# wpats/scanner

Hardware: AMD Instinct MI355X
Metric: Msamples/s (complex samples through convert->window->FFT->dB->threshold) (higher is better)
Workload: dtype f32

## Files before the change

scanner_amd/build.py:

```python
import os
import shutil
import subprocess
import sys

HERE = os.path.dirname(os.path.abspath(__file__))
CSRC = os.path.join(HERE, "csrc")
LIB = os.path.join(HERE, "libscanner_hip.so")
SOURCES = ["scn_kernels.hip", "scn_mixed.hip", "scn_generic.hip", "scn_big.hip", "scn_hits.hip", "scn_floor.hip", "scn_floor_local.hip", "scn_baseline.hip", "scn_welch.hip", "scn_average.hip", "scn_gather.hip", "scn_host.hip", "scn_plan.hip", "scn_submit.hip",
           "scn_collect.hip", "scn_welch_plan.hip"]
HEADERS = ["scn_kernels.h", "scn_mask.h", "scn_wire.h", "scn_dispatch.h", "scn_host.h", "scn_plan.h", "scn_resource.h", "scn_device.h", "scn_detect.h", "scn_mixed_dft.h", "scn_mixed_plans.h", "scn_sizes.h", "scn_gather_protocol.h", os.path.join("..", "..", "include", "scanner_hip.h")]
ARCH = "gfx950"
EXTRA_FLAGS = ["-fvisibility=hidden", "-fvisibility-inlines-hidden", "-DSCN_BUILDING_LIBRARY"]
PUBLIC_HEADER = os.path.join(HERE, "..", "include", "scanner_hip.h")
MAP_FILE = os.path.join(HERE, "libscanner_hip.map")
LINK_FLAGS = ["-Wl,--version-script=" + MAP_FILE]


def declared_symbols():
    import re

    with open(PUBLIC_HEADER) as fh:
        text = re.sub(r"/\*.*?\*/", "", fh.read(), flags=re.S)
    return sorted(set(re.findall(r"\bSCN_API\b[^;{]*?\b(scn_\w+)\s*\(", text)))


def write_map():
    with open(MAP_FILE, "w") as fh:
        fh.write("{\n  global:\n" + "".join(f"    {n};\n" for n in declared_symbols()) + "  local:\n    *;\n};\n")
SPLIT = {"scn_kernels.hip": ("SCN_TU", 8), "scn_mixed.hip": ("SCN_MIXED_TU", 8), "scn_average.hip": ("SCN_AVG_TU", 4)}


def hipcc():
    exe = shutil.which("hipcc") or "/opt/rocm/bin/hipcc"
    if not os.path.exists(exe):
        raise RuntimeError("hipcc not found; the HIP path cannot be built")
    return exe


def source_hash():
    import hashlib

    h = hashlib.sha256()
    for f in sorted(SOURCES + HEADERS):
        with open(os.path.join(CSRC, f), "rb") as fh:
            h.update(f.encode() + b"\0" + fh.read())
    with open(os.path.abspath(__file__), "rb") as fh:
        h.update(b"build.py\0" + fh.read())
    return h.hexdigest()[:16]


HASH_FILE = LIB + ".hash"


def _stale():
    if not os.path.exists(LIB) or not os.path.exists(HASH_FILE):
        return True
    with open(HASH_FILE) as fh:
        return fh.read().strip() != source_hash()


def build(force=False, verbose=False, defines=(), out=None):
    target = out or LIB
    if not out and not force and not _stale():
        return LIB
    import fcntl

    with open(LIB + ".lock", "w") as lock:
        fcntl.flock(lock, fcntl.LOCK_EX)
        if not out and not force and not _stale():
            return LIB
        return _build_locked(target, verbose, defines, out)


def _build_locked(target, verbose, defines, out):
    built_from = source_hash()
    write_map()
    objs, cmds = [], []
    tag = "" if not out else "." + os.path.basename(out).replace(".so", "")
    units = [(src, None) for src in SOURCES if src not in SPLIT] + [(src, tu) for src, (_, count) in SPLIT.items() for tu in range(count)]
    for src, tu in sorted(units, key=lambda u: u[1] is None):
        suffix = tag + ("" if tu is None else f".tu{tu}") + ".o"
        obj = os.path.join(os.path.dirname(out) if out else CSRC, src.replace(".hip", suffix))
        cmd = [hipcc(), f"--offload-arch={ARCH}", "-O3", "-std=c++17", "-fPIC", "-Wall", "-Wno-unused-function", "-Wno-unused-const-variable",
               "-fno-slp-vectorize", *EXTRA_FLAGS, *[f"-D{d}" for d in defines], *([] if tu is None else [f"-D{SPLIT[src][0]}={tu}"]),
               "-c", os.path.join(CSRC, src), "-o", obj]
        if verbose:
            print(" ".join(cmd), file=sys.stderr)
        cmds.append(cmd)
        objs.append(obj)
    from concurrent.futures import ThreadPoolExecutor

    with ThreadPoolExecutor(max_workers=min(len(cmds), os.cpu_count() or 1)) as pool:
        list(pool.map(subprocess.check_call, cmds))
    cmd = [hipcc(), f"--offload-arch={ARCH}", "-shared", "-fPIC", *LINK_FLAGS, "-o", target] + objs + ["-ldl"]
    if verbose:
        print(" ".join(cmd), file=sys.stderr)
    subprocess.check_call(cmd)
    if not out:
        with open(HASH_FILE, "w") as fh:
            fh.write(built_from + "\n")
    return target


HOST = os.path.join(HERE, "host")
HOST_LIB = os.path.join(HERE, "libscanner_host.so")
HOST_DEMO = os.path.join(HOST, "scan_synth")
ABI_BENCH = os.path.join(HOST, "abi_bench")
HOST_SOURCES = ["frequencyTable.cpp", "messageQueue.cpp", "captureWriter.cpp", "signalSource.cpp", "syntheticSource.cpp", "fileSource.cpp",
                "processInterface.cpp", "sampleBuffer.cpp", "process.cpp"]


def build_host(force=False, verbose=False):
    build(force=False)
    srcs = [os.path.join(HOST, f) for f in HOST_SOURCES]
    deps = srcs + [os.path.join(HOST, f) for f in os.listdir(HOST) if f.endswith(".h")] + [LIB]
    if force or not os.path.exists(HOST_LIB) or any(os.path.getmtime(d) > os.path.getmtime(HOST_LIB) for d in deps):
        cmd = ["g++", "-std=gnu++11", "-O2", "-g", "-fPIC", "-shared", "-Wall", "-pthread", "-o", HOST_LIB] + srcs + \
              ["-L" + HERE, "-lscanner_hip", "-Wl,-rpath,$ORIGIN"]
        if verbose:
            print(" ".join(cmd), file=sys.stderr)
        subprocess.check_call(cmd)
    demo_src = os.path.join(HOST, "scan_synth.cpp")
    if force or not os.path.exists(HOST_DEMO) or \
            max(os.path.getmtime(demo_src), os.path.getmtime(HOST_LIB)) > os.path.getmtime(HOST_DEMO):
        cmd = ["g++", "-std=gnu++11", "-O2", "-g", "-Wall", "-pthread", "-o", HOST_DEMO, demo_src, "-L" + HERE,
               "-lscanner_host", "-lscanner_hip", "-Wl,-rpath,$ORIGIN/.."]
        if verbose:
            print(" ".join(cmd), file=sys.stderr)
        subprocess.check_call(cmd)
    bench_src = os.path.join(HOST, "abi_bench.cpp")
    if force or not os.path.exists(ABI_BENCH) or os.path.getmtime(bench_src) > os.path.getmtime(ABI_BENCH) or \
            os.path.getmtime(os.path.join(HERE, "..", "include", "scanner_hip.h")) > os.path.getmtime(ABI_BENCH):
        rocm = os.environ.get("ROCM_PATH", "/opt/rocm")
        cmd = ["g++", "-std=gnu++11", "-O2", "-g", "-Wall", "-D__HIP_PLATFORM_AMD__", "-I" + os.path.join(rocm, "include"), "-o", ABI_BENCH,
               bench_src, "-L" + os.path.join(rocm, "lib"), "-lamdhip64", "-ldl", "-Wl,-rpath," + os.path.join(rocm, "lib")]
        if verbose:
            print(" ".join(cmd), file=sys.stderr)
        subprocess.check_call(cmd)
    return HOST_LIB, HOST_DEMO


if __name__ == "__main__":
    build_host(force="--force" in sys.argv, verbose=True)
    print(build(force="--force" in sys.argv, verbose=True))
```

scanner_amd/csrc/scn_kernels.hip:

```cpp
#include <hip/hip_runtime.h>
#include <hip/hip_ext.h>
#include <stdint.h>
#include <stdlib.h>

#include "scn_device.h"
#include "scn_dispatch.h"
#include "scn_kernels.h"

#ifndef SCN_TU
#define SCN_TU -1
#endif
#define SCN_IN_TU(x) (SCN_TU == -1 || SCN_TU == (x))
#define SCN_TU_COUNT 8


#define SCN_WORK_QUEUE_SETUP()                                                                         \
  const uint32_t wq_shard = blockIdx.x & 7u;                                                           \
  uint32_t *const wq_head = args.work_counter + 32u * wq_shard;        \
  const uint32_t wq_base = args.work_base[wq_shard];                                                   \
  const uint32_t wq_j0 = (gridDim.x - wq_shard + 7u) >> 3;                                             \
  uint32_t wq_zero;                                                                                    \
  asm("v_mov_b32 %0, 0" : "=v"(wq_zero));                                                              \
  auto wq_take = [&]() -> uint32_t { return atomicAdd(wq_head + wq_zero, 1u); };                       \
  auto wq_buffer = [&](uint32_t taken) -> uint32_t { return 8u * (wq_j0 + (taken - wq_base)) + wq_shard; }

template <int M, int KIND, bool DC, bool HITS, bool SPEC>
__global__ __launch_bounds__(16 * M, Geo<M>::WAVES_PER_SIMD) void scn_fft_kernel(ScnFftArgs args) {
  static_assert(HITS || SPEC, "a kernel that reports nothing");
  typedef Geo<M> G;
  constexpr int AUX_LD = SCN_AUX_LD;
  constexpr int AUX_ST = SCN_AUX_ST;
  constexpr bool DYN = scn_uses_queue(KIND, G::N);
  constexpr uint32_t N = G::N, T = G::T, P1 = G::P1, P2 = G::P2;
  typedef RawLoader<KIND> L;
  extern __shared__ __attribute__((aligned(16))) char smem_raw[];
  v2f *lds = reinterpret_cast<v2f *>(smem_raw);
  v2f *lds_tw2 = lds + G::EXCH;
  int *lds_cnt = reinterpret_cast<int *>(lds_tw2 + T);
  int *lds_hits = lds_cnt + 32;
  uint32_t *lds_next = reinterpret_cast<uint32_t *>(lds_hits + 2);

  const uint32_t t = threadIdx.x;
  const uint32_t p2 = t / M, c2 = t % M;
  const uint32_t lane = t & 63, wave = t >> 6;

  typename L::raw_t raw[16];
  if (blockIdx.x < args.n_buffers) {
    __amdgpu_buffer_rsrc_t r0 = make_rsrc(reinterpret_cast<const char *>(args.raw) + (size_t)blockIdx.x * L::kBytes * N, L::kBytes * N);
#pragma unroll
    for (int a = 0; a < 16; a++) raw[a] = L::template load<AUX_LD>(r0, N, t, T * a);
  }

  cf tw1[16];
#pragma unroll
  for (int p = 1; p < 16; p++) tw1[p] = from_v2f(args.tw1_table[(p - 1) * T + t]);
  float win[16];
#pragma unroll
  for (int a = 0; a < 16; a++) win[a] = args.window[T * a + t] * args.scale;
  lds_tw2[t] = args.twiddle[(16 * p2 * c2) & (N - 1)];
  SCN_WORK_QUEUE_SETUP();
  if (t == 0) {
    lds_hits[0] = lds_hits[1] = 0;
    lds_next[0] = DYN ? wq_buffer(wq_take()) : blockIdx.x + gridDim.x;
  }
  __syncthreads();

  v2f *w1 = lds + t;
  v2f *r1 = lds + p2 * P1 + c2;
  v2f *w2 = lds + c2 * P2 + p2;
  v2f *r3 = lds + t;
  const v2f *tw2 = lds_tw2 + c2;
  const uint32_t st_voff = t * 4u;

  auto joff_of = [](int o) -> uint32_t { return T * ((uint32_t)o / M) + 256u * ((uint32_t)o % M); };
  uint32_t keepmask = 0;
  if (HITS) {
#pragma unroll
    for (int o = 0; o < 16; o++) {
      const uint32_t j = t + joff_of(o);
      const uint32_t i = j ^ (N / 2);
      const bool keep = scn_bin_evaluated(j, i, N, args);
      keepmask |= keep ? (1u << o) : 0u;
    }
  }
  uint32_t par = 0;
  uint32_t prev = 0xffffffffu;

  uint32_t buf = blockIdx.x;
  uint32_t nxt = (uint32_t)__builtin_amdgcn_readfirstlane((int)lds_next[0]);
  while (buf < args.n_buffers) {
    const bool more = nxt < args.n_buffers;
    int dc_re = 0, dc_im = 0;
    if (DC) {
      int sr = 0, si = 0;
#pragma unroll
      for (int a = 0; a < 16; a++) {
        int re, im;
        L::ints(raw[a], re, im);
        sr += re;
        si += im;
      }
      sr = wave_sum(sr);
      si = wave_sum(si);
      if (lane == 0) {
        lds_cnt[wave] = sr;
        lds_cnt[16 + wave] = si;
      }
      __syncthreads();
      sr = si = 0;
#pragma unroll
      for (uint32_t w = 0; w < G::WAVES; w++) {
        sr += lds_cnt[w];
        si += lds_cnt[16 + w];
      }
      dc_re = (int)((uint32_t)sr / N);
      dc_im = (int)((uint32_t)si / N);
    }

    cf v[16];
#pragma unroll
    for (int a = 0; a < 16; a++) v[a] = L::conv(raw[a], dc_re, dc_im, 1.0f) * win[a];
    uint32_t taken = 0;
    if (DYN && t == 0 && more) taken = wq_take();
    const __amdgpu_buffer_rsrc_t rn =
        make_rsrc(reinterpret_cast<const char *>(args.raw) + (size_t)(more ? nxt : buf) * (L::kBytes * N), more ? L::kBytes * N : 0u);
    auto prefetch = [&](int a_lo, int a_hi) {
#pragma unroll
      for (int a = 0; a < 16; a++)
        if (a >= a_lo && a < a_hi) raw[a] = L::template load<AUX_LD>(rn, N, t, T * a);
    };
    prefetch(0, 6);

    fft16(v);
#pragma unroll
    for (int p = 0; p < 16; p++) {
      cf y = v[OUT16(p)];
      if (p) y = cmul(y, tw1[p]);
      w1[p * P1] = to_v2f(y);
    }
    __syncthreads();
    if (HITS) {
      if (t == 0 && prev != 0xffffffffu) {
        args.per_buffer_hits[prev] = (uint32_t)lds_hits[par ^ 1];
        if (args.host_hits) args.host_hits[prev] = (uint32_t)lds_hits[par ^ 1];
        lds_hits[par ^ 1] = 0;
      }
    }

#pragma unroll
    for (int b = 0; b < 16; b++) v[b] = from_v2f(r1[b * M]);
    prefetch(6, 11);
    fft16(v);
#pragma unroll
    for (int q = 1; q < 16; q++) v[OUT16(q)] = cmul(v[OUT16(q)], from_v2f(tw2[q * M]));
    __syncthreads();
    prefetch(11, 16);
#pragma unroll
    for (int q = 0; q < 16; q++) w2[q * 16] = to_v2f(v[OUT16(q)]);
    __syncthreads();

#pragma unroll
    for (int u = 0; u < 16 / M; u++)
#pragma unroll
      for (int c = 0; c < M; c++) v[u * M + c] = from_v2f(r3[c * P2 + T * u]);
    if constexpr (M == 16) fft16(v);
    if constexpr (M == 8) {
      fft8(v);
      fft8(v + 8);
    }
    if constexpr (M == 4) {
#pragma unroll
      for (int u = 0; u < 4; u++) radix4(v[4 * u], v[4 * u + 1], v[4 * u + 2], v[4 * u + 3]);
    }

    v16f pw;
    float gmax[4] = {0.0f, 0.0f, 0.0f, 0.0f};
    __amdgpu_buffer_rsrc_t rout = make_rsrc(args.power_db + (size_t)buf * N, (SPEC && args.power_db) ? 4u * N : 0u);
#pragma unroll
    for (int o = 0; o < 16; o++) {
      const float q = power_of(v[out_reg<M>(o)]);
      pw[o] = q;
      gmax[o >> 2] = fmaxf(gmax[o >> 2], q);
      if constexpr (SPEC) __builtin_amdgcn_raw_buffer_store_b32(__builtin_bit_cast(int, db_fast(q)), rout, st_voff, 4u * joff_of(o), AUX_ST);
    }
    const float pmax = fmaxf(fmaxf(gmax[0], gmax[1]), fmaxf(gmax[2], gmax[3]));
    if constexpr (SPEC) scn_store_exact_db<16>(pw, gmax, pmax, rout, st_voff, [&](int o) -> uint32_t { return 4u * joff_of(o); });
    if (t == 0) lds_next[0] = !more ? 0xffffffffu : DYN ? wq_buffer(taken) : nxt + gridDim.x;
    __syncthreads();
    const uint32_t after = (uint32_t)__builtin_amdgcn_readfirstlane((int)lds_next[0]);
    if (HITS) {
      if (__ballot(pmax > args.p_lo))
        scn_record_hits_lanes<16, false, true>(pw, gmax, keepmask, args, &lds_hits[par], buf, lane, [&](int o) -> uint32_t { return (t + joff_of(o)) ^ (N / 2); });
      prev = buf;
      par ^= 1;
    }
    buf = nxt;
    nxt = after;
  }
  if (HITS) {
    __syncthreads();
    if (t == 0 && prev != 0xffffffffu) {
      args.per_buffer_hits[prev] = (uint32_t)lds_hits[par ^ 1];
      if (args.host_hits) args.host_hits[prev] = (uint32_t)lds_hits[par ^ 1];
    }
  }
}

namespace {
template <int T, bool SPEC, bool HITS, typename POWER, typename JOFF, typename STORE>
__device__ __forceinline__ void scn_small_db_store_record(POWER power_at, JOFF joff_of, STORE store, const ScnFftArgs &args, uint32_t buf, bool valid,
                                                          uint32_t keepmask, uint32_t t, uint32_t n) {
  v16f pw, dbv;
  float gmax[4] = {0.0f, 0.0f, 0.0f, 0.0f};
#pragma unroll
  for (int o = 0; o < 16; o++) {
    const float q = power_at(o);
    pw[o] = q;
    gmax[o >> 2] = fmaxf(gmax[o >> 2], q);
    if constexpr (SPEC) {
      const float d = db_fast(q);
      dbv[o] = d;
      store(o, d, true);
    }
  }
  const float pmax = fmaxf(fmaxf(gmax[0], gmax[1]), fmaxf(gmax[2], gmax[3]));
  const bool any_cand = HITS && __ballot(valid && pmax > args.p_lo) != 0ull;
  if (SPEC || any_cand) {
    if constexpr (!SPEC) {
#pragma unroll
      for (int o = 0; o < 16; o++) dbv[o] = db_fast(pw[o]);
    }
    if (__ballot(pmax >= SCN_P_EXACT_FROM)) {
#pragma unroll
      for (int g = 0; g < 4; g++) {
        if (__ballot(gmax[g] >= SCN_P_EXACT_FROM)) {
#pragma unroll
          for (int o = 4 * g; o < 4 * g + 4; o++) {
            const float q = pw[o];
            if (__ballot(q >= SCN_P_EXACT_FROM)) {
              const float d = db_exact(q);
              dbv[o] = q >= SCN_P_EXACT_FROM ? d : dbv[o];
              if constexpr (SPEC) store(o, d, q >= SCN_P_EXACT_FROM);
            }
          }
        }
      }
    }
  }
  if constexpr (HITS) {
    uint32_t total = 0;
    if (any_cand) {
      uint32_t hm = 0;
#pragma unroll
      for (int o = 0; o < 16; o++) hm |= (dbv[o] > args.threshold) ? (1u << o) : 0u;
      hm &= valid ? keepmask : 0u;
      total = scn_record_hits_segment<T, 16>(dbv, hm, args, buf, t, [&](int o) -> uint32_t { return (t + joff_of(o)) ^ (n / 2); });
    }
    if (t == 0 && valid) {
      args.per_buffer_hits[buf] = total;
      if (args.host_hits) args.host_hits[buf] = total;
    }
  }
}

template <int M>
struct GeoSmall {
  static constexpr uint32_t N = 256u * M, T = 16u * M, SLOTS = 256u / T;
  static constexpr uint32_t P1 = T + M, P2 = 256u + 16u / M;
  static constexpr uint32_t EXCH = (16u * P1 > M * P2) ? 16u * P1 : M * P2;
  static constexpr uint32_t LDS_BYTES = SLOTS * EXCH * 8u + T * 8u + 16u;
  static constexpr uint32_t WG_PER_CU = 3;
};
}

template <int M, int KIND, bool DC, bool HITS, bool SPEC>
__global__ __launch_bounds__(256, 3) void scn_fft_small_kernel(ScnFftArgs args) {
  static_assert(M == 1 || M == 2, "256 or 512 points");
  static_assert(HITS || SPEC, "a kernel that reports nothing");
  typedef GeoSmall<M> G;
  constexpr int AUX_LD = SCN_AUX_LD;
  constexpr int AUX_ST = SCN_AUX_ST;
  constexpr uint32_t N = G::N, T = G::T, SLOTS = G::SLOTS, P1 = G::P1, P2 = G::P2;
  typedef RawLoader<KIND> L;
  extern __shared__ __attribute__((aligned(16))) char smem_raw[];
  const uint32_t tid = threadIdx.x, t = tid % T, slot = tid / T;
  v2f *lds = reinterpret_cast<v2f *>(smem_raw) + slot * G::EXCH;
  v2f *lds_tw2 = reinterpret_cast<v2f *>(smem_raw) + SLOTS * G::EXCH;
  const uint32_t p2 = t / M, c2 = t % M;
  const uint32_t buf_bytes = L::kBytes * N;

  auto in_rsrc = [&](uint32_t first) {
    const bool ok = first < args.n_buffers;
    const uint32_t nb = ok ? (args.n_buffers - first < SLOTS ? args.n_buffers - first : SLOTS) : 0u;
    return make_rsrc(reinterpret_cast<const char *>(args.raw) + (size_t)(ok ? first : 0u) * buf_bytes, nb * buf_bytes);
  };
  typename L::raw_t raw[16];
  auto load_group = [&](const __amdgpu_buffer_rsrc_t &r, int a_lo, int a_hi) {
#pragma unroll
    for (int a = 0; a < 16; a++)
      if (a >= a_lo && a < a_hi) raw[a] = L::template load<AUX_LD>(r, N, t + slot * (KIND == SCN_K_SHORT ? 2u * N : N), T * a);
  };
  uint32_t first = blockIdx.x * SLOTS;
  load_group(in_rsrc(first), 0, 16);

  cf tw1[16];
#pragma unroll
  for (int p = 1; p < 16; p++) tw1[p] = from_v2f(args.tw1_table[(p - 1) * T + t]);
  float win[16];
#pragma unroll
  for (int a = 0; a < 16; a++) win[a] = args.window[T * a + t] * args.scale;
  if (slot == 0) lds_tw2[t] = args.twiddle[(16 * p2 * c2) & (N - 1)];
  __syncthreads();

  v2f *w1 = lds + t;
  v2f *r1 = lds + p2 * P1 + c2;
  v2f *w2 = lds + c2 * P2 + p2;
  v2f *r3 = lds + t;
  const v2f *tw2 = lds_tw2 + c2;
  auto joff_of = [](int o) -> uint32_t { return T * ((uint32_t)o / M) + 256u * ((uint32_t)o % M); };
  uint32_t keepmask = 0;
  if (HITS) {
#pragma unroll
    for (int o = 0; o < 16; o++) {
      const uint32_t j = t + joff_of(o);
      const uint32_t i = j ^ (N / 2);
      const bool keep = scn_bin_evaluated(j, i, N, args);
      keepmask |= keep ? (1u << o) : 0u;
    }
  }

  for (; first < args.n_buffers; first += gridDim.x * SLOTS) {
    const uint32_t buf = first + slot;
    const bool valid = buf < args.n_buffers;
    int dc_re = 0, dc_im = 0;
    if (DC) {
      int sr = 0, si = 0;
#pragma unroll
      for (int a = 0; a < 16; a++) {
        int re, im;
        L::ints(raw[a], re, im);
        sr += re;
        si += im;
      }
#pragma unroll
      for (uint32_t off = T / 2; off > 0; off >>= 1) {
        sr += __shfl_xor(sr, (int)off, 64);
        si += __shfl_xor(si, (int)off, 64);
      }
      dc_re = (int)((uint32_t)sr / N);
      dc_im = (int)((uint32_t)si / N);
    }
    cf v[16];
#pragma unroll
    for (int a = 0; a < 16; a++) v[a] = L::conv(raw[a], dc_re, dc_im, 1.0f) * win[a];
    const __amdgpu_buffer_rsrc_t rn = in_rsrc(first + gridDim.x * SLOTS);
    load_group(rn, 0, 6);

    fft16(v);
#pragma unroll
    for (int p = 0; p < 16; p++) {
      cf y = v[OUT16(p)];
      if (p) y = cmul(y, tw1[p]);
      w1[p * P1] = to_v2f(y);
    }
    __syncthreads();
#pragma unroll
    for (int b = 0; b < 16; b++) v[b] = from_v2f(r1[b * M]);
    load_group(rn, 6, 11);
    fft16(v);
    if constexpr (M == 1) {
      load_group(rn, 11, 16);
    } else {
#pragma unroll
      for (int q = 1; q < 16; q++) v[OUT16(q)] = cmul(v[OUT16(q)], from_v2f(tw2[q * M]));
      __syncthreads();
      load_group(rn, 11, 16);
#pragma unroll
      for (int q = 0; q < 16; q++) w2[q * 16] = to_v2f(v[OUT16(q)]);
      __syncthreads();
#pragma unroll
      for (int u = 0; u < 16 / M; u++)
#pragma unroll
        for (int c = 0; c < M; c++) v[u * M + c] = from_v2f(r3[c * P2 + T * u]);
#pragma unroll
      for (int u = 0; u < 8; u++) {
        const cf a = v[2 * u], b = v[2 * u + 1];
        v[2 * u] = a + b;
        v[2 * u + 1] = a - b;
      }
    }
    const uint32_t nvalid = args.n_buffers - first < SLOTS ? args.n_buffers - first : SLOTS;
    __amdgpu_buffer_rsrc_t rout = make_rsrc(args.power_db + (size_t)first * N, (SPEC && args.power_db) ? nvalid * 4u * N : 0u);
    const uint32_t st_voff = (slot * N + t) * 4u;
    scn_small_db_store_record<(int)T, SPEC, HITS>(
        [&](int o) -> float { return power_of(v[M == 1 ? OUT16(o) : o]); }, joff_of,
        [&](int o, float d, bool pred) { __builtin_amdgcn_raw_buffer_store_b32(__builtin_bit_cast(int, d), rout, pred ? st_voff : 0x80000000u, 4u * joff_of(o), AUX_ST); },
        args, buf, valid, keepmask, t, N);
    __syncthreads();
  }
}

namespace {
template <int R>
struct GeoTiny {
  static constexpr uint32_t N = 16u * R, T = R, SLOTS = 256u / R;
  static constexpr uint32_t P1 = R + 1u;
  static constexpr uint32_t EXCH = R == 1 ? 0u : 16u * P1 + R;
  static constexpr uint32_t PITCH = N + R;
  static constexpr uint32_t TILE_BYTES = SLOTS * PITCH * 8u;
  static constexpr uint32_t LDS_BYTES = (TILE_BYTES > SLOTS * EXCH * 8u ? TILE_BYTES : SLOTS * EXCH * 8u) + 16u;
  static constexpr uint32_t WG_PER_CU = 3;
};

template <int KIND, int R>
struct TinyStage {
  typedef GeoTiny<R> G;
  typedef RawLoader<KIND> L;
  static constexpr bool PLANAR = KIND == SCN_K_SHORT;
  typedef typename L::raw_t reg_t;
  template <int AUX>
  static __device__ __forceinline__ reg_t load(__amdgpu_buffer_rsrc_t r, uint32_t tid, int a) {
    if constexpr (PLANAR) {
      return __builtin_amdgcn_raw_buffer_load_b32(r, tid * 4u, 1024u * (uint32_t)a, AUX);
    } else {
      return L::template load<AUX>(r, G::N, tid, 256u * (uint32_t)a);
    }
  }
  static __device__ __forceinline__ void stage(char *tile, uint32_t tid, int a, reg_t v) {
    if constexpr (PLANAR) {
      unsigned short *t16 = reinterpret_cast<unsigned short *>(tile);
#pragma unroll
      for (int h = 0; h < 2; h++) {
        const uint32_t e = 512u * (uint32_t)a + 2u * tid + h, s = e / (2u * G::N), j = e % (2u * G::N);
        t16[s * 2u * G::PITCH + (j < G::N ? j : G::PITCH + j - G::N)] = (unsigned short)(h ? (uint32_t)v >> 16 : (uint32_t)v & 0xffffu);
      }
    } else {
      const uint32_t e = 256u * (uint32_t)a + tid, idx = (e / G::N) * G::PITCH + e % G::N;
      if constexpr (KIND == SCN_K_FLOAT_COMPLEX) reinterpret_cast<v2f *>(tile)[idx] = v;
      else if constexpr (KIND == SCN_K_SHORT_COMPLEX) reinterpret_cast<int *>(tile)[idx] = v;
      else reinterpret_cast<unsigned short *>(tile)[idx] = (unsigned short)v;
    }
  }
  static __device__ __forceinline__ typename L::raw_t gather(const char *tile, uint32_t slot, uint32_t j) {
    if constexpr (PLANAR) {
      const unsigned short *t16 = reinterpret_cast<const unsigned short *>(tile) + slot * 2u * G::PITCH;
      return (int)((uint32_t)t16[j] | ((uint32_t)t16[G::PITCH + j] << 16));
    } else if constexpr (KIND == SCN_K_FLOAT_COMPLEX) {
      return reinterpret_cast<const v2f *>(tile)[slot * G::PITCH + j];
    } else if constexpr (KIND == SCN_K_SHORT_COMPLEX) {
      return reinterpret_cast<const int *>(tile)[slot * G::PITCH + j];
    } else {
      return (int)reinterpret_cast<const unsigned short *>(tile)[slot * G::PITCH + j];
    }
  }
};
}

template <int R, int KIND, bool DC, bool HITS, bool SPEC>
__global__ __launch_bounds__(256, 3) void scn_fft_tiny_kernel(ScnFftArgs args) {
// ... 924 lines not shown
```

Measured before the change: 459,200.

## Load float-complex samples in 16-byte pairs and swap halves with DPP

For float-complex input with M=16, the initial raw load now fetches two adjacent samples per lane with a 16-byte load (load2), using a permuted lane-to-sample mapping. Partner lanes then exchange halves through a DPP cndmask quad_perm swap so each lane ends up holding its original strided samples. The goal is wider, fewer memory transactions on the first buffer. By default the pairing is off inside the steady-state loop, so only the first buffer per block uses it, at the cost of extra cross-lane instructions and some inline-asm complexity.

```diff
diff --git a/scanner_amd/build.py b/scanner_amd/build.py
--- a/scanner_amd/build.py
+++ b/scanner_amd/build.py
@@ -8,7 +8,7 @@
 LIB = os.path.join(HERE, "libscanner_hip.so")
 SOURCES = ["scn_kernels.hip", "scn_mixed.hip", "scn_generic.hip", "scn_big.hip", "scn_hits.hip", "scn_floor.hip", "scn_floor_local.hip", "scn_baseline.hip", "scn_welch.hip", "scn_average.hip", "scn_gather.hip", "scn_host.hip", "scn_plan.hip", "scn_submit.hip",
            "scn_collect.hip", "scn_welch_plan.hip"]
-HEADERS = ["scn_kernels.h", "scn_mask.h", "scn_wire.h", "scn_dispatch.h", "scn_host.h", "scn_plan.h", "scn_resource.h", "scn_device.h", "scn_detect.h", "scn_mixed_dft.h", "scn_mixed_plans.h", "scn_sizes.h", "scn_gather_protocol.h", os.path.join("..", "..", "include", "scanner_hip.h")]
+HEADERS = ["scn_kernels.h", "scn_mask.h", "scn_wire.h", "scn_dispatch.h", "scn_host.h", "scn_plan.h", "scn_resource.h", "scn_device.h", "scn_detect.h", "scn_mixed_dft.h", "scn_mixed_plans.h", "scn_sizes.h", "scn_gather_protocol.h", "scn_pair_map.h", os.path.join("..", "..", "include", "scanner_hip.h")]
 ARCH = "gfx950"
 EXTRA_FLAGS = ["-fvisibility=hidden", "-fvisibility-inlines-hidden", "-DSCN_BUILDING_LIBRARY"]
 PUBLIC_HEADER = os.path.join(HERE, "..", "include", "scanner_hip.h")
diff --git a/scanner_amd/csrc/scn_kernels.hip b/scanner_amd/csrc/scn_kernels.hip
--- a/scanner_amd/csrc/scn_kernels.hip
+++ b/scanner_amd/csrc/scn_kernels.hip
@@ -2,10 +2,12 @@
 #include <hip/hip_ext.h>
 #include <stdint.h>
 #include <stdlib.h>
+#include <type_traits>
 
 #include "scn_device.h"
 #include "scn_dispatch.h"
 #include "scn_kernels.h"
+#include "scn_pair_map.h"
 
 #ifndef SCN_TU
 #define SCN_TU -1
@@ -24,6 +26,36 @@
   auto wq_take = [&]() -> uint32_t { return atomicAdd(wq_head + wq_zero, 1u); };                       \
   auto wq_buffer = [&](uint32_t taken) -> uint32_t { return 8u * (wq_j0 + (taken - wq_base)) + wq_shard; }
 
+__device__ __forceinline__ void scn_pair_swap_words(float &lx, float &ly, float &hx, float &hy, unsigned long long even_lanes) {
+  float ox, oy, px, py;
+  asm("s_mov_b64 vcc, %8\n\t"
+      "s_nop 0\n\t"
+      "v_cndmask_b32_dpp %0, %6, %4, vcc quad_perm:[1,0,3,2] row_mask:0xf bank_mask:0xf\n\t"
+      "v_cndmask_b32_dpp %1, %7, %5, vcc quad_perm:[1,0,3,2] row_mask:0xf bank_mask:0xf\n\t"
+      "s_not_b64 vcc, vcc\n\t"
+      "v_cndmask_b32_dpp %2, %4, %6, vcc quad_perm:[1,0,3,2] row_mask:0xf bank_mask:0xf\n\t"
+      "v_cndmask_b32_dpp %3, %5, %7, vcc quad_perm:[1,0,3,2] row_mask:0xf bank_mask:0xf"
+      : "=&v"(ox), "=&v"(oy), "=&v"(px), "=&v"(py)
+      : "v"(lx), "v"(ly), "v"(hx), "v"(hy), "s"(even_lanes)
+      : "vcc", "scc");
+  lx = ox;
+  ly = oy;
+  hx = px;
+  hy = py;
+}
+template <typename RAW>
+__device__ __forceinline__ void scn_pair_swap(RAW (&raw)[16]) {
+  if constexpr (sizeof(RAW) == 8) {
+#pragma unroll
+    for (int i = 0; i < scn_pair::LOADS; i++) {
+      float lx = raw[2 * i].x, ly = raw[2 * i].y, hx = raw[2 * i + 1].x, hy = raw[2 * i + 1].y;
+      scn_pair_swap_words(lx, ly, hx, hy, 0x5555555555555555ull);
+      raw[2 * i] = RAW{lx, ly};
+      raw[2 * i + 1] = RAW{hx, hy};
+    }
+  }
+}
+
 template <int M, int KIND, bool DC, bool HITS, bool SPEC>
 __global__ __launch_bounds__(16 * M, Geo<M>::WAVES_PER_SIMD) void scn_fft_kernel(ScnFftArgs args) {
   static_assert(HITS || SPEC, "a kernel that reports nothing");
@@ -32,6 +64,8 @@
   constexpr int AUX_ST = SCN_AUX_ST;
   constexpr bool DYN = scn_uses_queue(KIND, G::N);
   constexpr uint32_t N = G::N, T = G::T, P1 = G::P1, P2 = G::P2;
+  constexpr bool PAIR = KIND == SCN_K_FLOAT_COMPLEX && scn_pair::enabled(M);
+  constexpr bool PAIR_LOOP = PAIR && scn_pair::in_loop(M);
   typedef RawLoader<KIND> L;
   extern __shared__ __attribute__((aligned(16))) char smem_raw[];
   v2f *lds = reinterpret_cast<v2f *>(smem_raw);
@@ -45,10 +79,23 @@
   const uint32_t lane = t & 63, wave = t >> 6;
 
   typename L::raw_t raw[16];
+  const uint32_t pair_unit = scn_pair::lane_unit(T, t);
+  auto fetch = [&](const __amdgpu_buffer_rsrc_t &r, auto pair, int g_lo, int g_hi) {
+    if constexpr (decltype(pair)::value) {
+#pragma unroll
+      for (int i = 0; i < scn_pair::LOADS; i++)
+        if (i >= scn_pair::group_begin(g_lo) && i < scn_pair::group_begin(g_hi))
+          L::template load2<AUX_LD>(r, N, pair_unit, scn_pair::load_sample0(T, i), raw[2 * i], raw[2 * i + 1]);
+    } else {
+      constexpr int A[4] = {0, 6, 11, 16};
+#pragma unroll
+      for (int a = 0; a < 16; a++)
+        if (a >= A[g_lo] && a < A[g_hi]) raw[a] = L::template load<AUX_LD>(r, N, t, T * a);
+    }
+  };
   if (blockIdx.x < args.n_buffers) {
     __amdgpu_buffer_rsrc_t r0 = make_rsrc(reinterpret_cast<const char *>(args.raw) + (size_t)blockIdx.x * L::kBytes * N, L::kBytes * N);
-#pragma unroll
-    for (int a = 0; a < 16; a++) raw[a] = L::template load<AUX_LD>(r0, N, t, T * a);
+    fetch(r0, std::integral_constant<bool, PAIR>(), 0, 3);
   }
 
   cf tw1[16];
@@ -117,6 +164,11 @@
       dc_im = (int)((uint32_t)si / N);
     }
 
+    if constexpr (PAIR_LOOP) {
+      scn_pair_swap(raw);
+    } else if constexpr (PAIR) {
+      if (buf == blockIdx.x) scn_pair_swap(raw);
+    }
     cf v[16];
 #pragma unroll
     for (int a = 0; a < 16; a++) v[a] = L::conv(raw[a], dc_re, dc_im, 1.0f) * win[a];
@@ -124,12 +176,7 @@
     if (DYN && t == 0 && more) taken = wq_take();
     const __amdgpu_buffer_rsrc_t rn =
         make_rsrc(reinterpret_cast<const char *>(args.raw) + (size_t)(more ? nxt : buf) * (L::kBytes * N), more ? L::kBytes * N : 0u);
-    auto prefetch = [&](int a_lo, int a_hi) {
-#pragma unroll
-      for (int a = 0; a < 16; a++)
-        if (a >= a_lo && a < a_hi) raw[a] = L::template load<AUX_LD>(rn, N, t, T * a);
-    };
-    prefetch(0, 6);
+    fetch(rn, std::integral_constant<bool, PAIR_LOOP>(), 0, 1);
 
     fft16(v);
 #pragma unroll
@@ -149,12 +196,12 @@
 
 #pragma unroll
     for (int b = 0; b < 16; b++) v[b] = from_v2f(r1[b * M]);
-    prefetch(6, 11);
+    fetch(rn, std::integral_constant<bool, PAIR_LOOP>(), 1, 2);
     fft16(v);
 #pragma unroll
     for (int q = 1; q < 16; q++) v[OUT16(q)] = cmul(v[OUT16(q)], from_v2f(tw2[q * M]));
     __syncthreads();
-    prefetch(11, 16);
+    fetch(rn, std::integral_constant<bool, PAIR_LOOP>(), 2, 3);
 #pragma unroll
     for (int q = 0; q < 16; q++) w2[q * 16] = to_v2f(v[OUT16(q)]);
     __syncthreads();
diff --git a/scanner_amd/csrc/scn_pair_map.h b/scanner_amd/csrc/scn_pair_map.h
--- /dev/null
+++ b/scanner_amd/csrc/scn_pair_map.h
@@ -0,0 +1,46 @@
+#ifndef SCN_PAIR_MAP_H
+#define SCN_PAIR_MAP_H
+#include <stdint.h>
+
+namespace scn_pair {
+
+constexpr int LOADS = 8;
+
+constexpr uint32_t parity(uint32_t t) { return t & 1u; }
+constexpr uint32_t partner(uint32_t t) { return t ^ 1u; }
+constexpr uint32_t first_col(uint32_t t) { return t & ~1u; }
+
+constexpr uint32_t row(uint32_t par, int i) { return 2u * (uint32_t)i + par; }
+
+constexpr uint32_t lane_unit(uint32_t T, uint32_t t) { return (T / 2u) * parity(t) + (t >> 1); }
+constexpr uint32_t load_sample0(uint32_t T, int i) { return 2u * T * (uint32_t)i; }
+constexpr uint32_t load_byte(uint32_t T, uint32_t t, int i) { return 16u * lane_unit(T, t) + 8u * load_sample0(T, i); }
+constexpr uint32_t load_sample(uint32_t T, uint32_t t, int i, int h) { return T * row(parity(t), i) + first_col(t) + (uint32_t)h; }
+
+constexpr int kept_half(uint32_t par) { return (int)par; }
+constexpr int sent_half(uint32_t par) { return (int)(par ^ 1u); }
+constexpr int kept_reg(uint32_t par, int i) { return (int)row(par, i); }
+constexpr int recv_reg(uint32_t par, int i) { return (int)row(par ^ 1u, i); }
+
+#ifndef SCN_PAIR_SPLIT_1
+#define SCN_PAIR_SPLIT_1 3
+#endif
+#ifndef SCN_PAIR_SPLIT_2
+#define SCN_PAIR_SPLIT_2 6
+#endif
+constexpr int GROUPS = 3;
+constexpr int group_begin(int g) { return g <= 0 ? 0 : g == 1 ? SCN_PAIR_SPLIT_1 : g == 2 ? SCN_PAIR_SPLIT_2 : LOADS; }
+static_assert(0 <= SCN_PAIR_SPLIT_1 && SCN_PAIR_SPLIT_1 <= SCN_PAIR_SPLIT_2 && SCN_PAIR_SPLIT_2 <= LOADS, "the groups partition the loads");
+
+#ifndef SCN_FLOAT_PAIR_LOADS
+#define SCN_FLOAT_PAIR_LOADS 0x10
+#endif
+#ifndef SCN_FLOAT_PAIR_LOOP
+#define SCN_FLOAT_PAIR_LOOP 0
+#endif
+constexpr bool mask_has(int mask, int M) { return (M == 4 || M == 8 || M == 16) && ((mask >> (M == 4 ? 2 : M == 8 ? 3 : 4)) & 1) != 0; }
+constexpr bool enabled(int M) { return mask_has(SCN_FLOAT_PAIR_LOADS, M); }
+constexpr bool in_loop(int M) { return enabled(M) && mask_has(SCN_FLOAT_PAIR_LOOP, M); }
+
+}
+#endif
```

After: 459,600, median of 2. No clear change (+0.1%).
